# Sachin-A/TraceWeaver

Hardware: NVIDIA H100
Metric: spans/sec reconstructed (in+out spans of all solved services) (higher is better)
Workload: dtype int64 timestamps, f64 log-likelihoods

## Files before the change

### traceweaver_b200/csrc/tw_api.cu

```cuda
#include <cuda_runtime.h>

#include <cstdio>
#include <cstdlib>
#include <cstring>
#include <memory>
#include <random>
#include <string>
#include <vector>

#include "tw_kernels.cuh"

using namespace tw;

static thread_local std::string g_last_error;

static int fail(int code, const char* fmt, const char* a = "", const char* b2 = "") {
  char buf[512];
  snprintf(buf, sizeof buf, fmt, a, b2);
  g_last_error = buf;
  return code;
}

#define CU(expr)                                                                      \
  do {                                                                                \
// ... 52 lines not shown
  DevBuf<int32_t> truth_tab;
  DevBuf<int64_t> truth_tab_off;
  DevBuf<int32_t> in_prob;
  DevBuf<int> order_missing;
  DevBuf<uint8_t> acc_flags;
  DevBuf<unsigned long long> acc_first;
  DevBuf<uint32_t> skip_sets;
  DevBuf<int64_t> skip_set_off;
  DevBuf<uint32_t> skip_taken;
  DevBuf<int32_t> skip_win;
  DevBuf<int32_t> unit_prob;
  DevBuf<int32_t> unit_lo;
  DevBuf<int32_t> unit_hi;
  DevBuf<int> unit_count;
  int max_units = 0;
  DevBuf<int32_t> long_seg;
  int n_long = 0;
  DevBuf<int64_t> long_scratch;
  int64_t slab_len = 1;
  DevBuf<int64_t> in_end_sorted;
  DevBuf<int64_t> out_end_sorted;
  DevBuf<int32_t> batch_prob;
  DevBuf<int32_t> batch_idx;
  int n_batches_total = 0;
  DevBuf<int32_t> term_ep;
  DevBuf<int32_t> ep_prob;
  bool shifted = false;
  DevBuf<int64_t> fixed_times;
  DevBuf<int32_t> prob_shift;
  DevBuf<int32_t> prob_top;
// ... 186 lines not shown
  CU(up(eng->term_ep.p, term_ep));
  CU(up(eng->ep_prob.p, ep_prob));
  CU(cudaStreamSynchronize(s));

  {
    int64_t mu = 0;
    for (int p = 0; p < P; ++p) mu += (h->prob_in_off[p + 1] - h->prob_in_off[p]) / kStitchUnitMin + 1;
    if (mu > 0x7fffffff) return fail(TW_ERR_RANGE_LIMIT, "bind: too many stitch units");
    eng->max_units = (int)mu;
    CU(eng->unit_prob.reserve((size_t)mu));
    CU(eng->unit_lo.reserve((size_t)mu));
    CU(eng->unit_hi.reserve((size_t)mu));
    CU(eng->unit_count.reserve(1));
  }
  {
    std::vector<int32_t> long_seg;
    int64_t longest = 0;
    for (int p = 0; p < P; ++p) {
      const int64_t n = h->prob_in_off[p + 1] - h->prob_in_off[p];
      if (n > kSortSmemCap) { long_seg.push_back(p); longest = n > longest ? n : longest; }
    }
    for (int ep = 0; ep < h->n_ep_total; ++ep) {
      const int64_t n = h->ep_out_off[ep + 1] - h->ep_out_off[ep];
      if (n > kSortSmemCap) { long_seg.push_back(P + ep); longest = n > longest ? n : longest; }
      if (n > eng->max_seg) eng->max_seg = (int)n;
    }
    if (longest > (int64_t)1 << 28) return fail(TW_ERR_RANGE_LIMIT, "bind: a list has more than 2^28 spans");
    eng->n_long = (int)long_seg.size();
    eng->slab_len = 1;
    while (eng->slab_len < longest) eng->slab_len <<= 1;
// ... 333 lines not shown
    return fail(TW_ERR_INVALID, "tw_stitch: params, cut, assign, mis_rank, n_cand are required");
  if (out->topk_score && (!out->topk_idx || !out->topk_cnt)) return fail(TW_ERR_INVALID, "tw_stitch: partial topk outputs");
  tw_score_out spec;
  memset(&spec, 0, sizeof spec);
  if (undeleted) {
    if (!undeleted->topk_score || !undeleted->topk_idx || !undeleted->topk_cnt || !undeleted->n_feasible ||
        !undeleted->used_lo || !undeleted->used_bits || !undeleted->used_wide)
      return fail(TW_ERR_INVALID, "tw_stitch: `undeleted` needs top-K, n_feasible and the used maps");
    spec = *undeleted;
  }
  tw_params sp;
  rc = scoring_params(eng, params, sp, (cudaStream_t)stream);
  if (rc) return rc;
  StitchUnits ub{eng->unit_prob.p, eng->unit_lo.p, eng->unit_hi.p, eng->unit_count.p};
  CU(launch_stitch(eng->dev, sp, cut, spec, *out, eng->taken.p, eng->taken_words, eng->node_limit, ub,
                   eng->max_units, eng->err_flag.p, (cudaStream_t)stream, eng->launches));
  return TW_OK;
}

int tw_delays(tw_engine* eng, const int32_t* assign, const int64_t* term_sample_off, double* delays,
              int32_t* counts, void* stream) {
  int rc = need_bound(eng, "tw_delays");
  if (rc) return rc;
  CU(launch_delays(eng->dev, assign, term_sample_off, eng->term_ep.p, eng->ep_prob.p, delays, counts,
                   eng->shifted ? eng->prob_shift.p : nullptr, (cudaStream_t)stream, eng->launches));
  return TW_OK;
}

static void numpy_random_samples(uint32_t seed, int count, std::vector<double>& out) {
  std::mt19937 mt(seed);
  out.resize(count);
// ... 78 lines not shown
```

### traceweaver_b200/csrc/tw_core.cuh

```cuda
#pragma once
#include <stdint.h>
#include <string.h>
#include <math.h>

#include "../../include/traceweaver_b200.h"

#if defined(__CUDACC__)
#define TW_HD __host__ __device__ __forceinline__
#define TW_HD_NOINLINE __host__ __device__
#else
#define TW_HD inline
#define TW_HD_NOINLINE
#endif

#define TW_MAX_TERMS 48
#define TW_LOG_SQRT_2PI 0.91893853320467274178032973640562
#define TW_LOG_2PI 1.8378770664093453

namespace tw {

#if defined(__CUDA_ARCH__)
TW_HD double dmul(double a, double b) { return __dmul_rn(a, b); }
TW_HD double dadd(double a, double b) { return __dadd_rn(a, b); }
TW_HD double dsub(double a, double b) { return __dsub_rn(a, b); }
// ... 533 lines not shown
    int ai = wi + ws;
    if (ai >= W) break;
    uint32_t a = A[ai] >> bs;
    if (bs && ai + 1 < W) a |= A[ai + 1] << (32 - bs);
    if (a & B[wi]) return true;
  }
  return false;
}

struct WindowBuf {
  double score[TW_WINDOW_CAP][TW_K];
  int idx[TW_WINDOW_CAP][TW_K][TW_MAX_E];
  int cnt[TW_WINDOW_CAP];
  int chosen[TW_WINDOW_CAP];
  uint32_t adj[TW_WINDOW_CAP];
};

TW_HD bool tuples_conflict(const int* a, const int* b, int E) {
  for (int e = 0; e < E; ++e)
    if (a[e] == b[e]) return true;
  return false;
}

TW_HD uint32_t window_adjacency(const WindowBuf& wb, int E, int nw, int k) {
  uint32_t m = 0;
  for (int a = 0; a < nw; ++a) {
    if (a == k) continue;
    bool hit = false;
    for (int r = 0; r < wb.cnt[k] && !hit; ++r)
      for (int q = 0; q < wb.cnt[a] && !hit; ++q)
        hit = tuples_conflict(wb.idx[k][r], wb.idx[a][q], E);
    if (hit) m |= 1u << a;
  }
  return m;
}

#define TW_ASSIGN_MAX_COLS (TW_WINDOW_CAP * (TW_K + 1) + 1)
constexpr int kMwisPricedMin = 7;
constexpr int kMwisSimpleBudget = 1024;
TW_HD_NOINLINE inline void assignment_solve(const WindowBuf& wb, const int* member, int m, int pos, int* best,
                                            double (*price)[TW_K], double* price_total) {
  int colid[TW_WINDOW_CAP * TW_K];
  int ncol = 0;
  short ecol[TW_WINDOW_CAP][TW_K];
  for (int l = 0; l < m; ++l) {
    const int k = member[l];
    for (int r = 0; r < TW_K; ++r) {
      ecol[l][r] = -1;
      if (r >= wb.cnt[k] || !(TW_WEIGHT_OFFSET + wb.score[k][r] > 0.0)) continue;
      const int span = wb.idx[k][r][pos];
      int j = 0;
      while (j < ncol && colid[j] != span) ++j;
      if (j == ncol) colid[ncol++] = span;
      ecol[l][r] = (short)(j + 1);
    }
  }
  const int M = ncol + m;
  double u[TW_WINDOW_CAP + 1], vv[TW_ASSIGN_MAX_COLS], minv[TW_ASSIGN_MAX_COLS];
  short p[TW_ASSIGN_MAX_COLS], way[TW_ASSIGN_MAX_COLS];
  bool used[TW_ASSIGN_MAX_COLS];
  for (int i = 0; i <= m; ++i) u[i] = 0.0;
  for (int j = 0; j <= M; ++j) { vv[j] = 0.0; p[j] = 0; way[j] = 0; }
  const double INF = 1e300;
  for (int i = 1; i <= m; ++i) {
    p[0] = (short)i;
// ... 107 lines not shown
          } else {
            p[freed] = (short)(l + 1);
          }
        }
      }
      if (ok) {
        fixedc[j] = true;
        best[l] = r < TW_K ? r : -1;
        break;
      }
    }
  }
}

#define TW_MWIS_MAX_DEFERRED 4
TW_HD_NOINLINE inline long long mwis_solve(WindowBuf& wb, int E, int nw, long long node_limit,
                                           uint32_t* deferred = nullptr, int* n_deferred = nullptr) {
  long long nodes = 0;
  if (n_deferred) *n_deferred = 0;
  uint32_t todo = nw >= 32 ? 0xffffffffu : ((1u << nw) - 1u);
  for (int k = 0; k < nw; ++k) wb.chosen[k] = -1;
  while (todo) {
    int seed = 0;
    while (!(todo >> seed & 1u)) ++seed;
    uint32_t comp = 1u << seed, frontier = comp;
    while (frontier) {
      int k = 0;
      while (!(frontier >> k & 1u)) ++k;
      frontier &= ~(1u << k);
      uint32_t nb = wb.adj[k] & ~comp;
      comp |= nb;
// ... 56 lines not shown
        }
        int r = iter[level]++;
        if (r > wb.cnt[k]) { --level; continue; }
        if (r == wb.cnt[k]) {
          choice[level] = -1;
          cur[level + 1] = cur[level];
          ++level;
          iter[level] = 0;
          continue;
        }
        double w = TW_WEIGHT_OFFSET + wb.score[k][r];
        if (!(w > 0.0)) continue;
        bool ok = true;
        for (int l = 0; l < level && ok; ++l)
          if (choice[l] >= 0 && (wb.adj[k] >> member[l] & 1u) &&
              tuples_conflict(wb.idx[k][r], wb.idx[member[l]][choice[l]], E))
            ok = false;
        if (!ok) continue;
        choice[level] = r;
        cur[level + 1] = cur[level] + w;
        ++level;
        iter[level] = 0;
      }

      if (simple_done) {
        for (int l = 0; l < m; ++l) wb.chosen[member[l]] = best[l];
        continue;
      }
    }
    if (deferred && *n_deferred < TW_MWIS_MAX_DEFERRED) {
      deferred[(*n_deferred)++] = comp;
// ... 1 lines not shown
    }
#ifdef __CUDA_ARCH__
    return -1;
#else
    uint8_t avail[TW_WINDOW_CAP + 1][TW_WINDOW_CAP];
    double rem[TW_WINDOW_CAP + 1];
    double price[TW_WINDOW_CAP][TW_K];
    double remp[TW_WINDOW_CAP + 1], lam[TW_WINDOW_CAP + 1];
    const bool priced = m >= kMwisPricedMin;
    if (priced) {
      int pos = 0, fewest = 0x7fffffff;
      for (int e = 0; e < E; ++e) {
        int distinct = 0;
        for (int l = 0; l < m; ++l)
          for (int r = 0; r < wb.cnt[member[l]]; ++r) {
            const int sp = wb.idx[member[l]][r][e];
            bool seen = false;
            for (int l2 = 0; l2 <= l && !seen; ++l2)
              for (int r2 = 0; r2 < (l2 < l ? wb.cnt[member[l2]] : r) && !seen; ++r2)
                seen = wb.idx[member[l2]][r2][e] == sp;
            distinct += !seen;
          }
        if (distinct < fewest) { fewest = distinct; pos = e; }
      }
      assignment_solve(wb, member, m, pos, nullptr, price, &lam[0]);
      nodes += m;
    } else {
      lam[0] = 0.0;
      for (int l = 0; l < m; ++l)
        for (int r = 0; r < TW_K; ++r) price[l][r] = 0.0;
    }
    auto best_avail = [&](int j, uint8_t mask) {
      if (!mask) return 0.0;
      int r = 0;
      while (!(mask >> r & 1u)) ++r;
// ... 58 lines not shown
        rem[level + 1] = rem[level] - best_avail(level, avail[level][level]);
        remp[level + 1] = remp[level] - best_reduced(level, avail[level][level]);
        lam[level + 1] = lam[level];
        ++level;
        iter[level] = 0;
        continue;
      }
      if (!(avail[level][level] >> r & 1u)) continue;
      const double w = TW_WEIGHT_OFFSET + wb.score[k][r];
      double rest = 0.0, restp = 0.0;
      for (int j = level + 1; j < m; ++j) {
        uint8_t mask = avail[level][j];
        if (mask && (wb.adj[k] >> member[j] & 1u)) {
          const int kj = member[j];
          for (int q = 0; q < wb.cnt[kj]; ++q)
            if ((mask >> q & 1u) && tuples_conflict(wb.idx[k][r], wb.idx[kj][q], E)) mask &= (uint8_t)~(1u << q);
        }
        avail[level + 1][j] = mask;
        rest += best_avail(j, mask);
        if (priced) restp += best_reduced(j, mask);
      }
      choice[level] = r;
      cur[level + 1] = cur[level] + w;
      rem[level + 1] = rest;
      remp[level + 1] = restp;
      lam[level + 1] = lam[level] - price[level][r];
      ++level;
      iter[level] = 0;
    }
    for (int l = 0; l < m; ++l) wb.chosen[member[l]] = best[l];
#endif
// ... 22 lines not shown
```

### traceweaver_b200/csrc/tw_kernels.cuh

```cuda
#pragma once
#include <cuda_runtime.h>
#include <stdint.h>

#include "tw_core.cuh"

namespace tw {

constexpr int kS3Threads = 128;
constexpr int kS3Tile = 128;
constexpr int kStageSpans = 1536;
constexpr int kTblCap = 3072;
#ifndef TW_WARP_TBL_CAP
#define TW_WARP_TBL_CAP 256
#endif
constexpr int kWarpTblCap = TW_WARP_TBL_CAP;
constexpr int kRedoCoopCombos = 256;
constexpr int kStitchCoopCombos = 512;
constexpr int kTakenWords = 256;
constexpr int kNarrowW = 2;
constexpr int kWideW = 64;
constexpr int kWideThreads = 32;

constexpr int kStitchWarps = 2;

struct TileList {
  const int32_t* tile_prob;
  const int32_t* tile_start;
  int n_tiles;
  int tile_len;
  const int32_t* tile_cnt = nullptr;
};

struct ScoreTiles {
  const int32_t* tile_prob;
  const int32_t* tile_start;
  const int32_t* tile_win;
  uint8_t* overflow;
  int n_tiles;
// ... 18 lines not shown
cudaError_t launch_cut(const tw_batch& b, const tw_score_out& out, const ScoreTiles& st, const int32_t* prev_idx,
                       cudaStream_t s, int64_t& launches);
cudaError_t launch_score_redo(const tw_batch& b, const tw_params* prm, const tw_score_out& out,
                              const TileList& wide, const int32_t* prev_idx, uint8_t* tile_overflow,
                              int n_sm, int* err_flag, cudaStream_t s, int64_t& launches);
struct StitchUnits {
  int32_t* prob;
  int32_t* lo;
  int32_t* hi;
  int* count;
};
constexpr int kStitchUnitMin = 48;
constexpr int kStitchUnitMaxServices = 4096;
cudaError_t launch_stitch(const tw_batch& b, const tw_params& prm, const uint8_t* cut,
                          const tw_score_out& spec, const tw_pass_out& out, uint32_t* taken_words, size_t taken_n_words,
                          long long node_limit, const StitchUnits& unit_buf, int max_units, int* err_flag,
                          cudaStream_t s, int64_t& launches);
constexpr int kSortSmemCap = 16384;
cudaError_t launch_sort_ends(const tw_batch& b, int64_t* in_end_sorted, int64_t* out_end_sorted,
                             int max_seg, const int32_t* long_seg, int n_long, int64_t* long_scratch,
                             int64_t slab_len, int* err_flag, cudaStream_t s, int64_t& launches);
cudaError_t launch_params0(const tw_batch& b, const int64_t* in_end_sorted,
                           const int64_t* out_end_sorted, const int64_t* prob_gauss_off,
                           const int32_t* batch_prob, const int32_t* batch_idx, int n_batches_total,
                           double* gauss_out, const int32_t* prob_shift, cudaStream_t s, int64_t& launches);
cudaError_t launch_delays(const tw_batch& b, const int32_t* assign, const int64_t* term_sample_off,
                          const int32_t* term_ep, const int32_t* ep_prob, double* delays,
                          int32_t* counts, const int32_t* prob_shift, cudaStream_t s, int64_t& launches);

constexpr int kShiftInvalid = 1 << 30;
constexpr int kFixedBits = 55;
struct TimesF64 {
// ... 64 lines not shown
```

### traceweaver_b200/csrc/tw_stitch.cu

```cuda
#include "tw_kernels.cuh"

namespace tw {

#ifdef TW_PROFILE_PHASES
__device__ unsigned long long g_stitch_phase[16];
#define TW_SPHASE(k)                                                                 \
  do {                                                                               \
    if (lane == 0) {                                                                 \
      long long _now = clock64();                                                    \
      atomicAdd(&g_stitch_phase[k], (unsigned long long)(_now - _sp_t0));            \
      _sp_t0 = _now;                                                                 \
    }                                                                                \
  } while (0)
#define TW_SCOUNT(k, v) do { if (lane == 0) atomicAdd(&g_stitch_phase[k], (unsigned long long)(v)); } while (0)
#else
#define TW_SPHASE(k) do { } while (0)
#define TW_SCOUNT(k, v) do { } while (0)
#endif

__device__ __forceinline__ void prefetch_l1(const void* p) {
  asm volatile("prefetch.global.L1 [%0];" ::"l"(p));
}

struct StitchWarpSmem {
  ProbView v;
  WindowBuf wb;
  double tbl[kWarpTblCap];
  uint32_t tk[kTakenWords];
  uint32_t tmp[kTakenWords];
  uint8_t sid[kWarpTblCap];
  uint32_t cconf[32];
  double cw[32];
};

constexpr int kSmallWindow = 6;
constexpr int kSmallSpace = 4096;
__device__ __forceinline__ bool stitch_small_window(StitchWarpSmem& sm, int E, int nw, int lane, long long* nodes_out) {
  WindowBuf& wb = sm.wb;
  const unsigned kAll = 0xffffffffu;
  const int k = lane / TW_K, r = lane - TW_K * k;
  const bool valid = k < nw && r < wb.cnt[k];
  const unsigned vmask = __ballot_sync(kAll, valid);
  uint32_t conf = 0u;
  if (valid) {
    for (int e = 0; e < E; ++e) conf |= __match_any_sync(vmask, wb.idx[k][r][e]);
    conf &= ~(0x1fu << (TW_K * k));
  }
  sm.cconf[lane] = conf;
  sm.cw[lane] = valid ? TW_WEIGHT_OFFSET + wb.score[k][r] : 0.0;
  uint32_t am = 0u;
#pragma unroll
  for (int a = 0; a < kSmallWindow; ++a)
    if ((conf >> (TW_K * a)) & 0x1fu) am |= 1u << a;
  if (lane < nw) { wb.adj[lane] = 0u; wb.chosen[lane] = -1; }
  __syncwarp();
  if (am) atomicOr(&wb.adj[k], am);
  __syncwarp();
  int cnt[kSmallWindow];
  uint32_t adj[kSmallWindow];
#pragma unroll
// ... 71 lines not shown
      for (int a = 0; a < kSmallWindow; ++a) {
        if ((comp >> a) & 1u) {
          const int d = rem / stride[a];
          rem -= d * stride[a];
          if (lane == 0) wb.chosen[a] = d < cnt[a] ? d : -1;
        }
      }
    }
    nodes += space;
  }
  *nodes_out = nodes;
  return true;
}


__device__ __noinline__ long long mwis_component_warp(WindowBuf& wb, int E, uint32_t comp, double* price ,
                                                      long long node_limit, long long nodes, int lane) {
  const unsigned kAll = 0xffffffffu;
  const int m = __popc(comp);
  int kmine = -1;
  {
    uint32_t c = comp;
    for (int l = 0; l < m; ++l) {
      const int k = __ffs(c) - 1;
      c &= c - 1u;
      if (l == lane) kmine = k;
    }
  }
  double lam0 = 0.0;
  if (lane == 0) {
    int member[TW_WINDOW_CAP];
    {
      uint32_t c = comp;
      for (int l = 0; l < m; ++l) { member[l] = __ffs(c) - 1; c &= c - 1u; }
    }
    int pos = 0, fewest = 0x7fffffff;
    for (int e = 0; e < E; ++e) {
      int distinct = 0;
      for (int l = 0; l < m; ++l)
        for (int r = 0; r < wb.cnt[member[l]]; ++r) {
          const int sp = wb.idx[member[l]][r][e];
          bool seen = false;
          for (int l2 = 0; l2 <= l && !seen; ++l2)
            for (int r2 = 0; r2 < (l2 < l ? wb.cnt[member[l2]] : r) && !seen; ++r2)
              seen = wb.idx[member[l2]][r2][e] == sp;
          distinct += !seen;
        }
      if (distinct < fewest) { fewest = distinct; pos = e; }
    }
    assignment_solve(wb, member, m, pos, nullptr, reinterpret_cast<double(*)[TW_K]>(price), &lam0);
  }
  __syncwarp();
  lam0 = __shfl_sync(kAll, lam0, 0);
  nodes += m;
  const bool mine = lane < m;
  const int cnt = mine ? wb.cnt[kmine] : 0;
  double w0 = 0, w1 = 0, w2 = 0, w3 = 0, w4 = 0, q0 = 0, q1 = 0, q2 = 0, q3 = 0, q4 = 0;
  uint8_t av[TW_WINDOW_CAP + 1];
  {
    uint8_t mask = 0;
// ... 62 lines not shown
      if (lane == level) myc = -1;
      av[level + 1] = avmine;
      cur[level + 1] = cur[level];
      rem[level + 1] = rem[level] - ob;
      remp[level + 1] = remp[level] - obp;
      lam[level + 1] = lam[level];
      ++level;
      iter[level] = 0;
      continue;
    }
    if (!(avL >> r & 1u)) continue;
    const int kL = __shfl_sync(kAll, kmine, level);
    uint8_t mask = avmine;
    if (mine && lane > level && mask && (wb.adj[kL] >> kmine & 1u)) {
      for (int q = 0; q < cnt; ++q)
        if ((mask >> q & 1u) && tuples_conflict(wb.idx[kL][r], wb.idx[kmine][q], E)) mask &= (uint8_t)~(1u << q);
    }
    av[level + 1] = mask;
    const bool later = mine && lane > level;
    const double rest = wsum(later ? best_avail(mask) : 0.0);
    const double restp = wsum(later ? best_reduced(mask) : 0.0);
    if (lane == level) myc = r;
    cur[level + 1] = cur[level] + (TW_WEIGHT_OFFSET + wb.score[kL][r]);
    rem[level + 1] = rest;
    remp[level + 1] = restp;
    lam[level + 1] = lam[level] - price[level * TW_K + r];
    ++level;
    iter[level] = 0;
  }
  if (mine) wb.chosen[kmine] = bestc;
  __syncwarp();
  return nodes;
}

__device__ __noinline__ void stitch_search_lanes(StitchWarpSmem& sm, const tw_params& prm, const tw_pass_out& out,
                                                 uint32_t* const* tk_base, const OutWin* w,
                                                 const double* gauss_base, const double* mix_base, const double* etab,
                                                 int E, int lane, int ws, int i, int64_t in_s, int64_t in_e,
                                                 bool todo, int batch0) {
  const ProbView& v = sm.v;
  WindowBuf& wb = sm.wb;
  auto is_taken = [&](int e, int o) {
    return (reinterpret_cast<volatile const uint32_t*>(tk_base[e])[o >> 5] >> (o & 31)) & 1u;
  };
  const bool active = todo, fast = false;
  int lo[TW_MAX_E], r[TW_MAX_E], lo_abs[TW_MAX_E];
  int tsize = 0;
  if (active && !fast) {
    for (int e = 0; e < E; ++e) {
      lo[e] = lower_bound(w[e].s, w[e].n, in_s);
      lo_abs[e] = lo[e];
      r[e] = range_len(w[e], lo[e], in_e);
    }
    tsize = term_table_size(v, r);
  }
  const int brel = i / TW_PARAM_BATCH - batch0;
  auto publish = [&](const TopK& tk, int leaves) {
    const int64_t gi = v.in_off + i;
    out.n_cand[gi] = leaves;
    wb.cnt[lane] = tk.n;
    for (int k = 0; k < tk.n; ++k) {
      wb.score[lane][k] = tk.score[k];
      for (int e = 0; e < E; ++e) wb.idx[lane][k][e] = tk.idx[k][e];
    }
    if (out.topk_score) {
      out.topk_cnt[gi] = (uint8_t)tk.n;
      int32_t* ix = out.topk_idx + TW_K * (v.tuple_off + (int64_t)i * E);
      for (int k = 0; k < TW_K; ++k) {
        out.topk_score[gi * TW_K + k] = k < tk.n ? tk.score[k] : __longlong_as_double(0x7ff8000000000000LL);
        for (int e = 0; e < E; ++e) ix[k * E + e] = k < tk.n ? tk.idx[k][e] : -1;
      }
    }
  };
  bool pending = active;
  {
    const long long Pown = pending ? combo_count(v, r) : 0;
    unsigned heavy = __ballot_sync(0xffffffffu, pending && tsize <= kWarpTblCap && Pown > kStitchCoopCombos &&
                                                    Pown < (1LL << 31));
    while (heavy) {
      const int L = __ffs(heavy) - 1;
      heavy &= heavy - 1u;
      int lo_b[TW_MAX_E], r_b[TW_MAX_E], o_last_b[TW_MAX_E];
      for (int e = 0; e < E; ++e) {
        lo_b[e] = __shfl_sync(0xffffffffu, lo[e], L);
        r_b[e] = __shfl_sync(0xffffffffu, r[e], L);
      }
      const int tsz = __shfl_sync(0xffffffffu, tsize, L);
      const int brel_b = __shfl_sync(0xffffffffu, brel, L);
      const long long P_b = __shfl_sync(0xffffffffu, Pown, L);
      term_table_last_offsets(v, r_b, o_last_b);
      if (lane == L) term_table_fill(v, in_s, in_e, w, lo, r, o_last_b, brel_b, is_taken, sm.tbl, sm.sid);
      __syncwarp();
      for (int sl = lane; sl < tsz; sl += 32) {
        const uint8_t id = sm.sid[sl];
        if (id != TW_SLOT_INVALID) {
          ParamView pv;
          pv.mode = prm.mode;
          pv.gauss = gauss_base ? gauss_base + (int64_t)(batch0 + (id >> 6)) * v.n_terms * TW_GAUSS_REC : nullptr;
          pv.mix = mix_base;
          pv.etab = etab;
          sm.tbl[sl] = term_logpdf(pv, id & 63, sm.tbl[sl]);
        }
      }
      __syncwarp();
      TopK part;
      part.clear();
      int leaves = 0;
      bool tie = false;
      enumerate_combos(v, w, lo_b, r_b, o_last_b, sm.sid, lane, 32, P_b,
                       [&](const int* c, const int64_t* ce, long long) {
                         ++leaves;
                         const double sc = table_score(v, r_b, lo_b, sm.tbl, c, ce);
                         for (int k = 0; k < part.n; ++k) tie = tie || part.score[k] == sc;
                         tie = tie || sc != sc;
                         topk_offer_sorted(v, part, sc, c);
                       });
#pragma unroll
      for (int d = 16; d > 0; d >>= 1) leaves += __shfl_xor_sync(0xffffffffu, leaves, d);
      TopK tkc;
      tkc.clear();
      int head = 0;
      double prev = 0.0;
      for (int round = 0; round <= TW_K; ++round) {
        const double hs = head < part.n ? part.score[head] : -INFINITY;
        double mx = hs;
#pragma unroll
        for (int d = 16; d > 0; d >>= 1) {
// ... 27 lines not shown
    int my = pending ? tsize : 0, incl = my;
#pragma unroll
    for (int d = 1; d < 32; d <<= 1) {
      int o = __shfl_up_sync(0xffffffffu, incl, d);
      if (lane >= d) incl += o;
    }
    const int offset = incl - my;
    const bool lazy = pending && offset == 0 && tsize > kWarpTblCap;
    const bool in_round = pending && !lazy && offset + tsize <= kWarpTblCap;
    int total = in_round ? offset + tsize : 0;
#pragma unroll
    for (int d = 16; d > 0; d >>= 1) total = max(total, __shfl_xor_sync(0xffffffffu, total, d));
    int o_last[TW_MAX_E];
    if (in_round) {
      term_table_last_offsets(v, r, o_last);
      term_table_fill(v, in_s, in_e, w, lo, r, o_last, brel, is_taken, sm.tbl + offset, sm.sid + offset);
    }
    if (lazy) {
      ParamView pv;
      pv.mode = prm.mode;
      pv.gauss = gauss_base ? gauss_base + (int64_t)(i / TW_PARAM_BATCH) * v.n_terms * TW_GAUSS_REC : nullptr;
      pv.mix = mix_base;
      pv.etab = etab;
      TopK tk;
      tk.clear();
      int leaves = 0;
      enumerate(v, in_s, in_e, w, lo, is_taken,
                [&](const int* c, const int64_t* cs, const int64_t* ce) {
                  if (leaves < 0x7fffffff) ++leaves;
                  topk_offer(v, tk, score_tuple(v, pv, in_s, in_e, cs, ce), c);
                });
      topk_finish(v, tk);
      publish(tk, leaves);
      pending = false;
    }
    __syncwarp();
    for (int s = lane; s < total; s += 32) {
      const uint8_t id = sm.sid[s];
      if (id != TW_SLOT_INVALID) {
        ParamView pv;
        pv.mode = prm.mode;
        pv.gauss = gauss_base ? gauss_base + (int64_t)(batch0 + (id >> 6)) * v.n_terms * TW_GAUSS_REC : nullptr;
        pv.mix = mix_base;
        pv.etab = etab;
        sm.tbl[s] = term_logpdf(pv, id & 63, sm.tbl[s]);
      }
    }
    __syncwarp();
    if (in_round) {
      const double* tbl = sm.tbl + offset;
      const uint8_t* sid = sm.sid + offset;
      TopK tk;
      tk.clear();
      int leaves = 0;
      enumerate(v, in_s, in_e, w, lo,
                [&](int e, int o) { return sid[o_last[e] + (o - lo_abs[e])] == TW_SLOT_INVALID; },
                [&](const int* c, const int64_t*, const int64_t* ce) {
                  if (leaves < 0x7fffffff) ++leaves;
                  topk_offer(v, tk, table_score(v, r, lo_abs, tbl, c, ce), c);
                });
      topk_finish(v, tk);
      publish(tk, leaves);
      pending = false;
    }
    if (!__any_sync(0xffffffffu, pending)) break;
    __syncwarp();
  }
  __syncwarp();

}

__device__ __noinline__ long long stitch_mwis_large(StitchWarpSmem& sm, int E, int nw, long long node_limit, int lane) {
  WindowBuf& wb = sm.wb;
  long long nodes = 1;
  __syncwarp();
  if (lane < nw) wb.adj[lane] = window_adjacency(wb, E, nw, lane);
  __syncwarp();
  uint32_t deferred[TW_MWIS_MAX_DEFERRED];
  int n_def = 0;
  if (lane == 0) nodes = mwis_solve(wb, E, nw, node_limit, deferred, &n_def);
  nodes = __shfl_sync(0xffffffffu, nodes, 0);
  n_def = __shfl_sync(0xffffffffu, n_def, 0);
  for (int d = 0; d < n_def && nodes >= 0; ++d) {
    const uint32_t comp = __shfl_sync(0xffffffffu, lane == 0 ? deferred[d] : 0u, 0);
    __syncwarp();
    nodes = mwis_component_warp(wb, E, comp, sm.tbl, node_limit, nodes, lane);
  }
  return nodes;
}

__global__ void __launch_bounds__(kStitchWarps * 32, 10)
k_stitch(tw_batch b, tw_params prm, const uint8_t* __restrict__ cut_all, tw_score_out spec, tw_pass_out out,
         uint32_t* __restrict__ taken, long long node_limit, StitchUnits units, int* __restrict__ err_flag) {
  extern __shared__ __align__(16) unsigned char smem_raw[];
  __shared__ double etab[64];
  load_exp_table(etab);
  const int warp_in_block = threadIdx.x >> 5;
  const int lane = threadIdx.x & 31;
  const int u = blockIdx.x * kStitchWarps + warp_in_block;
  int p, u0 = 0, u1 = -1;
  if (units.prob) {
    if (u >= *units.count) return;
    p = units.prob[u];
    u0 = units.lo[u];
    u1 = units.hi[u];
  } else {
    p = u;
    if (p >= b.n_problems) return;
  }
  StitchWarpSmem& sm = reinterpret_cast<StitchWarpSmem*>(smem_raw)[warp_in_block];
#ifdef TW_PROFILE_PHASES
  long long _sp_t0 = clock64();
#endif
  int rc = TW_OK;
  if (lane == 0) rc = load_view(b, p, sm.v);
  rc = __shfl_sync(0xffffffffu, rc, 0);
  __syncwarp();
  if (rc != TW_OK) {
    if (lane == 0) { atomicMin(err_flag, rc); if (out.counters) out.counters[p * 4 + 3] = rc; }
    return;
  }
  const ProbView& v = sm.v;
  WindowBuf& wb = sm.wb;
  const int n = v.n_in, E = v.E;
  if (u1 < 0) u1 = n;
  const uint8_t* cut = cut_all + v.in_off;

  uint32_t* tk_base[TW_MAX_E];
  OutWin w[TW_MAX_E];
  int tk_words = 0;
  for (int e = 0; e < E; ++e) tk_words += (v.n_out[e] >> 5) + 3;
  const bool tk_smem = tk_words <= kTakenWords;
  {
    int off = 0;
    for (int e = 0; e < E; ++e) {
      tk_base[e] = tk_smem ? sm.tk + off : taken + (v.out_off[e] >> 5) + (v.ep0 + e);
      off += (v.n_out[e] >> 5) + 3;
      w[e].s = v.os[e]; w[e].e = v.oe[e]; w[e].base = 0; w[e].n = v.n_out[e];
    }
  }
  if (tk_smem)
    for (int x = lane; x < tk_words; x += 32) { sm.tk[x] = 0u; sm.tmp[x] = 0u; }
  __syncwarp();
  for (int i = u0 + lane; i < u1; i += 32) {
    out.mis_rank[v.in_off + i] = -1;
    for (int e = 0; e < E; ++e) out.assign[v.tuple_off + (int64_t)e * n + i] = -1;
  }

  const double* gauss_base = prm.mode == TW_PARAMS_GAUSS_BATCHED
                                 ? prm.gauss + prm.prob_gauss_off[p] * TW_GAUSS_REC : nullptr;
  const double* mix_base = prm.mode == TW_PARAMS_MIXTURE ? prm.mix + (int64_t)v.term0 * TW_MIX_REC : nullptr;

  WindowCursor wc;
  wc.init();
  int not_best = 0, unassigned = 0;
  long long max_nodes = 0;
  int ws = u0;
// ... 31 lines not shown
        const bool act = lane < R;
        const int ir = ws + (act ? lane : 0);
        const int64_t gi = v.in_off + ir;
        const int64_t base = v.tuple_off + (int64_t)ir * E;
        bool ok = act ? spec.used_wide[gi] == 0 : true;
        if (act && ok) {
          for (int e = 0; e < E; ++e) {
            const int ulo = spec.used_lo[base + e];
            const uint32_t u0 = spec.used_bits[2 * (base + e)], u1 = spec.used_bits[2 * (base + e) + 1];
            if ((u0 | u1) == 0u) continue;
            const int q = ulo >> 5, sh = ulo & 31;
            const uint32_t m0 = u0 << sh;
            const uint32_t m1 = sh ? (u0 >> (32 - sh)) | (u1 << sh) : u1;
            const uint32_t m2 = sh ? (u1 >> (32 - sh)) : 0u;
            uint32_t* tkp = tk_base[e] + q;
            uint32_t* tmp = sm.tmp + (tkp - sm.tk);
            if ((tkp[0] & m0) | (tkp[1] & m1) | (tkp[2] & m2)) ok = false;
            if (m0 && (atomicOr(&tmp[0], m0) & m0)) ok = false;
            if (m1 && (atomicOr(&tmp[1], m1) & m1)) ok = false;
            if (m2 && (atomicOr(&tmp[2], m2) & m2)) ok = false;
          }
        }
        const bool all_ok = __all_sync(0xffffffffu, ok);
        __syncwarp();
        if (act && spec.used_wide[gi] == 0) {
          for (int e = 0; e < E; ++e) {
            const int ulo = spec.used_lo[base + e];
            uint32_t* tmp = sm.tmp + ((tk_base[e] + (ulo >> 5)) - sm.tk);
            tmp[0] = 0u; tmp[1] = 0u; tmp[2] = 0u;
          }
        }
        __syncwarp();
        TW_SPHASE(2);
        if (all_ok) {
          int rank = -2;
          if (act) {
            const int cnt = spec.topk_cnt[gi];
            rank = (cnt > 0 && TW_WEIGHT_OFFSET + spec.topk_score[gi * TW_K] > 0.0) ? 0 : -1;
            out.n_cand[gi] = spec.n_feasible[gi];
            out.mis_rank[gi] = (int8_t)rank;
            if (rank == 0) {
              const int32_t* ix = spec.topk_idx + TW_K * base;
              for (int e = 0; e < E; ++e) {
// ... 64 lines not shown
        const uint32_t a = tkw[0], bq = tkw[1], c2 = tkw[2];
        hit |= __funnelshift_r(a, bq, sh) & u0;
        hit |= __funnelshift_r(bq, c2, sh) & u1;
      }
      fast = hit == 0u;
    }
    const int batch0 = ws / TW_PARAM_BATCH;
    if (fast) {
      const int64_t gi = v.in_off + i;
      const int cnt = spec.topk_cnt[gi];
      out.n_cand[gi] = spec.n_feasible[gi];
      wb.cnt[lane] = cnt;
      const int32_t* ix = spec.topk_idx + TW_K * (v.tuple_off + (int64_t)i * E);
      for (int k = 0; k < cnt; ++k) {
        wb.score[lane][k] = spec.topk_score[gi * TW_K + k];
        for (int e = 0; e < E; ++e) wb.idx[lane][k][e] = ix[k * E + e];
      }
      if (out.topk_score) {
        out.topk_cnt[gi] = (uint8_t)cnt;
        int32_t* ox = out.topk_idx + TW_K * (v.tuple_off + (int64_t)i * E);
        for (int k = 0; k < TW_K; ++k) {
          out.topk_score[gi * TW_K + k] = spec.topk_score[gi * TW_K + k];
          for (int e = 0; e < E; ++e) ox[k * E + e] = ix[k * E + e];
        }
      }
    }
    TW_SPHASE(5);
    const unsigned slow_mask = __ballot_sync(0xffffffffu, active && !fast);
    TW_SCOUNT(14, __popc(slow_mask));
    if (slow_mask)
      stitch_search_lanes(sm, prm, out, tk_base, w, gauss_base, mix_base, etab, E, lane, ws, i, in_s, in_e,
                          active && !fast, batch0);
    __syncwarp();
    TW_SPHASE(6);
    long long nodes = 1;
    if (nw == 1) {
      if (lane == 0) wb.chosen[0] = (wb.cnt[0] > 0 && TW_WEIGHT_OFFSET + wb.score[0][0] > 0.0) ? 0 : -1;
    } else {
      bool solved = false;
      if (nw <= kSmallWindow) solved = stitch_small_window(sm, E, nw, lane, &nodes);
      if (!solved) {
        nodes = stitch_mwis_large(sm, E, nw, node_limit, lane);
      }
    }
    __syncwarp();
    TW_SPHASE(7);
    if (nodes < 0) { rc = TW_ERR_MWIS_LIMIT; break; }
    if (nodes > max_nodes) max_nodes = nodes;
    int rank = -2;
    if (lane < nw) {
      rank = wb.chosen[lane];
      out.mis_rank[v.in_off + i] = (int8_t)rank;
      if (rank >= 0) {
        for (int e = 0; e < E; ++e) {
          int o = wb.idx[lane][rank][e];
          out.assign[v.tuple_off + (int64_t)e * n + i] = o;
          atomicOr(&tk_base[e][o >> 5], 1u << (o & 31));
        }
      }
    }
    not_best += __popc(__ballot_sync(0xffffffffu, lane < nw && rank != 0));
    unassigned += __popc(__ballot_sync(0xffffffffu, lane < nw && rank < 0));
    if (!tk_smem) __threadfence_block();
    __syncwarp();
    ws = we + 1;
    TW_SPHASE(8);
  }
  if (lane == 0) {
    if (rc != TW_OK) atomicMin(err_flag, rc);
    if (out.counters) {
// ... 73 lines not shown
  emit(unit_start, n);
}

#ifdef TW_PROFILE_PHASES
extern "C" int tw_debug_stitch_phases(unsigned long long* out16, int reset) {
  cudaError_t e = cudaMemcpyFromSymbol(out16, g_stitch_phase, sizeof(unsigned long long) * 16);
  if (e != cudaSuccess) return -2;
  if (reset) {
    unsigned long long z[16] = {0};
    cudaMemcpyToSymbol(g_stitch_phase, z, sizeof z);
  }
  return 0;
}
#endif

cudaError_t setup_stitch() {
  return cudaFuncSetAttribute(k_stitch, cudaFuncAttributeMaxDynamicSharedMemorySize,
                              (int)(sizeof(StitchWarpSmem) * kStitchWarps));
}

cudaError_t launch_stitch(const tw_batch& b, const tw_params& prm, const uint8_t* cut,
                          const tw_score_out& spec, const tw_pass_out& out, uint32_t* taken_words, size_t taken_n_words,
                          long long node_limit, const StitchUnits& unit_buf, int max_units, int* err_flag,
                          cudaStream_t s, int64_t& launches) {
  cudaError_t e = cudaMemsetAsync(taken_words, 0, taken_n_words * sizeof(uint32_t), s);
  if (e != cudaSuccess) return e;
  if (out.counters) {
    e = cudaMemsetAsync(out.counters, 0, (size_t)b.n_problems * 4 * sizeof(int32_t), s);
    if (e != cudaSuccess) return e;
  }
  size_t smem = sizeof(StitchWarpSmem) * kStitchWarps;
  StitchUnits units{nullptr, nullptr, nullptr, nullptr};
  int warps = b.n_problems;
  if (spec.used_lo && unit_buf.prob && max_units > 0 && b.n_problems < kStitchUnitMaxServices) {
    units = unit_buf;
    e = cudaMemsetAsync(units.count, 0, sizeof(int), s);
    if (e != cudaSuccess) return e;
    k_stitch_units<<<(b.n_problems + 3) / 4, 128, 0, s>>>(b, cut, spec, kStitchUnitMin, units);
    e = after_launch(launches);
    if (e != cudaSuccess) return e;
    warps = max_units;
  }
  int blocks = (warps + kStitchWarps - 1) / kStitchWarps;
  k_stitch<<<blocks, kStitchWarps * 32, smem, s>>>(b, prm, cut, spec, out, taken_words, node_limit, units, err_flag);
  return after_launch(launches);
}

}
```

Baseline: 438.7 million.

## Shrink stitch shared memory with runtime-sized slabs and global scratch tables

The per-warp shared-memory block of the stitch kernel is reorganized. The term tables move to a global-memory scratch array, the taken/tmp bitmaps are sized from the bound workload, and the window buffer is repacked by endpoint so only the needed endpoint columns are allocated. Launch bounds now target more blocks per SM. The goal is higher occupancy on the latency-bound stitch kernel, at the cost of term-table accesses going to global memory and a possible register squeeze from the higher launch-bounds target.

Result: faster. 456.1 million, median of 6 (+4.0%).

```diff
diff --git a/traceweaver_b200/csrc/tw_api.cu b/traceweaver_b200/csrc/tw_api.cu
--- a/traceweaver_b200/csrc/tw_api.cu
+++ b/traceweaver_b200/csrc/tw_api.cu
@@ -90,6 +90,8 @@
   DevBuf<int32_t> unit_hi;
   DevBuf<int> unit_count;
   int max_units = 0;
+  StitchLayout stitch_layout{};
+  DevBuf<StitchTables> stitch_tables;
   DevBuf<int32_t> long_seg;
   int n_long = 0;
   DevBuf<int64_t> long_scratch;
@@ -306,6 +308,18 @@
     CU(eng->unit_count.reserve(1));
   }
   {
+    int e_max = 1, tk_max = 0;
+    for (int p = 0; p < P; ++p) {
+      const int ep0 = h->prob_ep_off[p], E = h->prob_ep_off[p + 1] - ep0;
+      int tk = 0;
+      for (int e = 0; e < E; ++e) tk += (int)((h->ep_out_off[ep0 + e + 1] - h->ep_out_off[ep0 + e]) >> 5) + 3;
+      e_max = E > e_max ? E : e_max;
+      tk_max = tk > tk_max ? tk : tk_max;
+    }
+    eng->stitch_layout = stitch_layout(e_max, tk_max);
+    CU(eng->stitch_tables.reserve((size_t)(P > eng->max_units ? P : eng->max_units) + kStitchWarps));
+  }
+  {
     std::vector<int32_t> long_seg;
     int64_t longest = 0;
     for (int p = 0; p < P; ++p) {
@@ -669,7 +683,8 @@
   if (rc) return rc;
   StitchUnits ub{eng->unit_prob.p, eng->unit_lo.p, eng->unit_hi.p, eng->unit_count.p};
   CU(launch_stitch(eng->dev, sp, cut, spec, *out, eng->taken.p, eng->taken_words, eng->node_limit, ub,
-                   eng->max_units, eng->err_flag.p, (cudaStream_t)stream, eng->launches));
+                   eng->max_units, eng->stitch_layout, eng->stitch_tables.p, eng->err_flag.p, (cudaStream_t)stream,
+                   eng->launches));
   return TW_OK;
 }
 
diff --git a/traceweaver_b200/csrc/tw_core.cuh b/traceweaver_b200/csrc/tw_core.cuh
--- a/traceweaver_b200/csrc/tw_core.cuh
+++ b/traceweaver_b200/csrc/tw_core.cuh
@@ -571,6 +571,21 @@
   int cnt[TW_WINDOW_CAP];
   int chosen[TW_WINDOW_CAP];
   uint32_t adj[TW_WINDOW_CAP];
+  TW_HD int& at(int k, int r, int e) { return idx[k][r][e]; }
+  TW_HD int at(int k, int r, int e) const { return idx[k][r][e]; }
+};
+
+struct PackedWindowBuf {
+  double score[TW_WINDOW_CAP][TW_K];
+  int cnt[TW_WINDOW_CAP];
+  int chosen[TW_WINDOW_CAP];
+  uint32_t adj[TW_WINDOW_CAP];
+  int idx[TW_MAX_E][TW_WINDOW_CAP * TW_K];
+  TW_HD int& at(int k, int r, int e) { return idx[e][k * TW_K + r]; }
+  TW_HD int at(int k, int r, int e) const { return idx[e][k * TW_K + r]; }
+  static constexpr int packed_bytes(int e_max) {
+    return (int)(sizeof(PackedWindowBuf) - sizeof(int) * TW_WINDOW_CAP * TW_K * (TW_MAX_E - e_max));
+  }
 };
 
 TW_HD bool tuples_conflict(const int* a, const int* b, int E) {
@@ -579,14 +594,22 @@
   return false;
 }
 
-TW_HD uint32_t window_adjacency(const WindowBuf& wb, int E, int nw, int k) {
+template <class WB>
+TW_HD bool cands_conflict(const WB& wb, int k, int r, int a, int q, int E) {
+  for (int e = 0; e < E; ++e)
+    if (wb.at(k, r, e) == wb.at(a, q, e)) return true;
+  return false;
+}
+
+template <class WB>
+TW_HD uint32_t window_adjacency(const WB& wb, int E, int nw, int k) {
   uint32_t m = 0;
   for (int a = 0; a < nw; ++a) {
     if (a == k) continue;
     bool hit = false;
     for (int r = 0; r < wb.cnt[k] && !hit; ++r)
       for (int q = 0; q < wb.cnt[a] && !hit; ++q)
-        hit = tuples_conflict(wb.idx[k][r], wb.idx[a][q], E);
+        hit = cands_conflict(wb, k, r, a, q, E);
     if (hit) m |= 1u << a;
   }
   return m;
@@ -595,7 +618,8 @@
 #define TW_ASSIGN_MAX_COLS (TW_WINDOW_CAP * (TW_K + 1) + 1)
 constexpr int kMwisPricedMin = 7;
 constexpr int kMwisSimpleBudget = 1024;
-TW_HD_NOINLINE inline void assignment_solve(const WindowBuf& wb, const int* member, int m, int pos, int* best,
+template <class WB>
+TW_HD_NOINLINE inline void assignment_solve(const WB& wb, const int* member, int m, int pos, int* best,
                                             double (*price)[TW_K], double* price_total) {
   int colid[TW_WINDOW_CAP * TW_K];
   int ncol = 0;
@@ -605,7 +629,7 @@
     for (int r = 0; r < TW_K; ++r) {
       ecol[l][r] = -1;
       if (r >= wb.cnt[k] || !(TW_WEIGHT_OFFSET + wb.score[k][r] > 0.0)) continue;
-      const int span = wb.idx[k][r][pos];
+      const int span = wb.at(k, r, pos);
       int j = 0;
       while (j < ncol && colid[j] != span) ++j;
       if (j == ncol) colid[ncol++] = span;
@@ -743,7 +767,8 @@
 }
 
 #define TW_MWIS_MAX_DEFERRED 4
-TW_HD_NOINLINE inline long long mwis_solve(WindowBuf& wb, int E, int nw, long long node_limit,
+template <class WB>
+TW_HD_NOINLINE inline long long mwis_solve(WB& wb, int E, int nw, long long node_limit,
                                            uint32_t* deferred = nullptr, int* n_deferred = nullptr) {
   long long nodes = 0;
   if (n_deferred) *n_deferred = 0;
@@ -830,7 +855,7 @@
         bool ok = true;
         for (int l = 0; l < level && ok; ++l)
           if (choice[l] >= 0 && (wb.adj[k] >> member[l] & 1u) &&
-              tuples_conflict(wb.idx[k][r], wb.idx[member[l]][choice[l]], E))
+              cands_conflict(wb, k, r, member[l], choice[l], E))
             ok = false;
         if (!ok) continue;
         choice[level] = r;
@@ -862,11 +887,11 @@
         int distinct = 0;
         for (int l = 0; l < m; ++l)
           for (int r = 0; r < wb.cnt[member[l]]; ++r) {
-            const int sp = wb.idx[member[l]][r][e];
+            const int sp = wb.at(member[l], r, e);
             bool seen = false;
             for (int l2 = 0; l2 <= l && !seen; ++l2)
               for (int r2 = 0; r2 < (l2 < l ? wb.cnt[member[l2]] : r) && !seen; ++r2)
-                seen = wb.idx[member[l2]][r2][e] == sp;
+                seen = wb.at(member[l2], r2, e) == sp;
             distinct += !seen;
           }
         if (distinct < fewest) { fewest = distinct; pos = e; }
@@ -955,7 +980,7 @@
         if (mask && (wb.adj[k] >> member[j] & 1u)) {
           const int kj = member[j];
           for (int q = 0; q < wb.cnt[kj]; ++q)
-            if ((mask >> q & 1u) && tuples_conflict(wb.idx[k][r], wb.idx[kj][q], E)) mask &= (uint8_t)~(1u << q);
+            if ((mask >> q & 1u) && cands_conflict(wb, k, r, kj, q, E)) mask &= (uint8_t)~(1u << q);
         }
         avail[level + 1][j] = mask;
         rest += best_avail(j, mask);
diff --git a/traceweaver_b200/csrc/tw_kernels.cuh b/traceweaver_b200/csrc/tw_kernels.cuh
--- a/traceweaver_b200/csrc/tw_kernels.cuh
+++ b/traceweaver_b200/csrc/tw_kernels.cuh
@@ -22,6 +22,19 @@
 constexpr int kWideThreads = 32;
 
 constexpr int kStitchWarps = 2;
+constexpr int kStitchBlocksPerSM = 14;
+
+struct StitchTables {
+  double tbl[kWarpTblCap];
+  uint8_t sid[kWarpTblCap];
+};
+
+struct StitchLayout {
+  int tk_words;
+  int wb_off;
+  int bytes;
+};
+StitchLayout stitch_layout(int e_max, int tk_words_max);
 
 struct TileList {
   const int32_t* tile_prob;
@@ -70,8 +83,8 @@
 constexpr int kStitchUnitMaxServices = 4096;
 cudaError_t launch_stitch(const tw_batch& b, const tw_params& prm, const uint8_t* cut,
                           const tw_score_out& spec, const tw_pass_out& out, uint32_t* taken_words, size_t taken_n_words,
-                          long long node_limit, const StitchUnits& unit_buf, int max_units, int* err_flag,
-                          cudaStream_t s, int64_t& launches);
+                          long long node_limit, const StitchUnits& unit_buf, int max_units, const StitchLayout& layout,
+                          StitchTables* tables, int* err_flag, cudaStream_t s, int64_t& launches);
 constexpr int kSortSmemCap = 16384;
 cudaError_t launch_sort_ends(const tw_batch& b, int64_t* in_end_sorted, int64_t* out_end_sorted,
                              int max_seg, const int32_t* long_seg, int n_long, int64_t* long_scratch,
diff --git a/traceweaver_b200/csrc/tw_stitch.cu b/traceweaver_b200/csrc/tw_stitch.cu
--- a/traceweaver_b200/csrc/tw_stitch.cu
+++ b/traceweaver_b200/csrc/tw_stitch.cu
@@ -24,26 +24,31 @@
 
 struct StitchWarpSmem {
   ProbView v;
-  WindowBuf wb;
-  double tbl[kWarpTblCap];
-  uint32_t tk[kTakenWords];
-  uint32_t tmp[kTakenWords];
-  uint8_t sid[kWarpTblCap];
   uint32_t cconf[32];
   double cw[32];
 };
+static_assert(sizeof(StitchWarpSmem) % 8 == 0, "the taken bitmaps and the window buffer follow 8-byte aligned");
+
+struct StitchSlab {
+  unsigned char* base;
+  __device__ StitchWarpSmem& fixed() const { return *reinterpret_cast<StitchWarpSmem*>(base); }
+  __device__ uint32_t* taken() const { return reinterpret_cast<uint32_t*>(base + sizeof(StitchWarpSmem)); }
+  __device__ PackedWindowBuf& window(const StitchLayout& L) const {
+    return *reinterpret_cast<PackedWindowBuf*>(base + L.wb_off);
+  }
+};
 
 constexpr int kSmallWindow = 6;
 constexpr int kSmallSpace = 4096;
-__device__ __forceinline__ bool stitch_small_window(StitchWarpSmem& sm, int E, int nw, int lane, long long* nodes_out) {
-  WindowBuf& wb = sm.wb;
+__device__ __forceinline__ bool stitch_small_window(StitchWarpSmem& sm, PackedWindowBuf& wb, int E, int nw, int lane,
+                                                    long long* nodes_out) {
   const unsigned kAll = 0xffffffffu;
   const int k = lane / TW_K, r = lane - TW_K * k;
   const bool valid = k < nw && r < wb.cnt[k];
   const unsigned vmask = __ballot_sync(kAll, valid);
   uint32_t conf = 0u;
   if (valid) {
-    for (int e = 0; e < E; ++e) conf |= __match_any_sync(vmask, wb.idx[k][r][e]);
+    for (int e = 0; e < E; ++e) conf |= __match_any_sync(vmask, wb.at(k, r, e));
     conf &= ~(0x1fu << (TW_K * k));
   }
   sm.cconf[lane] = conf;
@@ -145,7 +150,7 @@
 }
 
 
-__device__ __noinline__ long long mwis_component_warp(WindowBuf& wb, int E, uint32_t comp, double* price ,
+__device__ __noinline__ long long mwis_component_warp(PackedWindowBuf& wb, int E, uint32_t comp, double* price ,
                                                       long long node_limit, long long nodes, int lane) {
   const unsigned kAll = 0xffffffffu;
   const int m = __popc(comp);
@@ -170,11 +175,11 @@
       int distinct = 0;
       for (int l = 0; l < m; ++l)
         for (int r = 0; r < wb.cnt[member[l]]; ++r) {
-          const int sp = wb.idx[member[l]][r][e];
+          const int sp = wb.at(member[l], r, e);
           bool seen = false;
           for (int l2 = 0; l2 <= l && !seen; ++l2)
             for (int r2 = 0; r2 < (l2 < l ? wb.cnt[member[l2]] : r) && !seen; ++r2)
-              seen = wb.idx[member[l2]][r2][e] == sp;
+              seen = wb.at(member[l2], r2, e) == sp;
           distinct += !seen;
         }
       if (distinct < fewest) { fewest = distinct; pos = e; }
@@ -267,7 +272,7 @@
     uint8_t mask = avmine;
     if (mine && lane > level && mask && (wb.adj[kL] >> kmine & 1u)) {
       for (int q = 0; q < cnt; ++q)
-        if ((mask >> q & 1u) && tuples_conflict(wb.idx[kL][r], wb.idx[kmine][q], E)) mask &= (uint8_t)~(1u << q);
+        if ((mask >> q & 1u) && cands_conflict(wb, kL, r, kmine, q, E)) mask &= (uint8_t)~(1u << q);
     }
     av[level + 1] = mask;
     const bool later = mine && lane > level;
@@ -286,13 +291,12 @@
   return nodes;
 }
 
-__device__ __noinline__ void stitch_search_lanes(StitchWarpSmem& sm, const tw_params& prm, const tw_pass_out& out,
+__device__ __noinline__ void stitch_search_lanes(const ProbView& v, PackedWindowBuf& wb, StitchTables& tb,
+                                                 const tw_params& prm, const tw_pass_out& out,
                                                  uint32_t* const* tk_base, const OutWin* w,
                                                  const double* gauss_base, const double* mix_base, const double* etab,
                                                  int E, int lane, int ws, int i, int64_t in_s, int64_t in_e,
                                                  bool todo, int batch0) {
-  const ProbView& v = sm.v;
-  WindowBuf& wb = sm.wb;
   auto is_taken = [&](int e, int o) {
     return (reinterpret_cast<volatile const uint32_t*>(tk_base[e])[o >> 5] >> (o & 31)) & 1u;
   };
@@ -314,7 +318,7 @@
     wb.cnt[lane] = tk.n;
     for (int k = 0; k < tk.n; ++k) {
       wb.score[lane][k] = tk.score[k];
-      for (int e = 0; e < E; ++e) wb.idx[lane][k][e] = tk.idx[k][e];
+      for (int e = 0; e < E; ++e) wb.at(lane, k, e) = tk.idx[k][e];
     }
     if (out.topk_score) {
       out.topk_cnt[gi] = (uint8_t)tk.n;
@@ -342,17 +346,17 @@
       const int brel_b = __shfl_sync(0xffffffffu, brel, L);
       const long long P_b = __shfl_sync(0xffffffffu, Pown, L);
       term_table_last_offsets(v, r_b, o_last_b);
-      if (lane == L) term_table_fill(v, in_s, in_e, w, lo, r, o_last_b, brel_b, is_taken, sm.tbl, sm.sid);
+      if (lane == L) term_table_fill(v, in_s, in_e, w, lo, r, o_last_b, brel_b, is_taken, tb.tbl, tb.sid);
       __syncwarp();
       for (int sl = lane; sl < tsz; sl += 32) {
-        const uint8_t id = sm.sid[sl];
+        const uint8_t id = tb.sid[sl];
         if (id != TW_SLOT_INVALID) {
           ParamView pv;
           pv.mode = prm.mode;
           pv.gauss = gauss_base ? gauss_base + (int64_t)(batch0 + (id >> 6)) * v.n_terms * TW_GAUSS_REC : nullptr;
           pv.mix = mix_base;
           pv.etab = etab;
-          sm.tbl[sl] = term_logpdf(pv, id & 63, sm.tbl[sl]);
+          tb.tbl[sl] = term_logpdf(pv, id & 63, tb.tbl[sl]);
         }
       }
       __syncwarp();
@@ -360,10 +364,10 @@
       part.clear();
       int leaves = 0;
       bool tie = false;
-      enumerate_combos(v, w, lo_b, r_b, o_last_b, sm.sid, lane, 32, P_b,
+      enumerate_combos(v, w, lo_b, r_b, o_last_b, tb.sid, lane, 32, P_b,
                        [&](const int* c, const int64_t* ce, long long) {
                          ++leaves;
-                         const double sc = table_score(v, r_b, lo_b, sm.tbl, c, ce);
+                         const double sc = table_score(v, r_b, lo_b, tb.tbl, c, ce);
                          for (int k = 0; k < part.n; ++k) tie = tie || part.score[k] == sc;
                          tie = tie || sc != sc;
                          topk_offer_sorted(v, part, sc, c);
@@ -421,7 +425,7 @@
     int o_last[TW_MAX_E];
     if (in_round) {
       term_table_last_offsets(v, r, o_last);
-      term_table_fill(v, in_s, in_e, w, lo, r, o_last, brel, is_taken, sm.tbl + offset, sm.sid + offset);
+      term_table_fill(v, in_s, in_e, w, lo, r, o_last, brel, is_taken, tb.tbl + offset, tb.sid + offset);
     }
     if (lazy) {
       ParamView pv;
@@ -443,20 +447,20 @@
     }
     __syncwarp();
     for (int s = lane; s < total; s += 32) {
-      const uint8_t id = sm.sid[s];
+      const uint8_t id = tb.sid[s];
       if (id != TW_SLOT_INVALID) {
         ParamView pv;
         pv.mode = prm.mode;
         pv.gauss = gauss_base ? gauss_base + (int64_t)(batch0 + (id >> 6)) * v.n_terms * TW_GAUSS_REC : nullptr;
         pv.mix = mix_base;
         pv.etab = etab;
-        sm.tbl[s] = term_logpdf(pv, id & 63, sm.tbl[s]);
+        tb.tbl[s] = term_logpdf(pv, id & 63, tb.tbl[s]);
       }
     }
     __syncwarp();
     if (in_round) {
-      const double* tbl = sm.tbl + offset;
-      const uint8_t* sid = sm.sid + offset;
+      const double* tbl = tb.tbl + offset;
+      const uint8_t* sid = tb.sid + offset;
       TopK tk;
       tk.clear();
       int leaves = 0;
@@ -477,8 +481,8 @@
 
 }
 
-__device__ __noinline__ long long stitch_mwis_large(StitchWarpSmem& sm, int E, int nw, long long node_limit, int lane) {
-  WindowBuf& wb = sm.wb;
+__device__ __noinline__ long long stitch_mwis_large(PackedWindowBuf& wb, StitchTables& tb, int E, int nw,
+                                                   long long node_limit, int lane) {
   long long nodes = 1;
   __syncwarp();
   if (lane < nw) wb.adj[lane] = window_adjacency(wb, E, nw, lane);
@@ -491,14 +495,15 @@
   for (int d = 0; d < n_def && nodes >= 0; ++d) {
     const uint32_t comp = __shfl_sync(0xffffffffu, lane == 0 ? deferred[d] : 0u, 0);
     __syncwarp();
-    nodes = mwis_component_warp(wb, E, comp, sm.tbl, node_limit, nodes, lane);
+    nodes = mwis_component_warp(wb, E, comp, tb.tbl, node_limit, nodes, lane);
   }
   return nodes;
 }
 
-__global__ void __launch_bounds__(kStitchWarps * 32, 10)
+__global__ void __launch_bounds__(kStitchWarps * 32, kStitchBlocksPerSM)
 k_stitch(tw_batch b, tw_params prm, const uint8_t* __restrict__ cut_all, tw_score_out spec, tw_pass_out out,
-         uint32_t* __restrict__ taken, long long node_limit, StitchUnits units, int* __restrict__ err_flag) {
+         uint32_t* __restrict__ taken, long long node_limit, StitchUnits units, StitchLayout layout,
+         StitchTables* __restrict__ tables, int* __restrict__ err_flag) {
   extern __shared__ __align__(16) unsigned char smem_raw[];
   __shared__ double etab[64];
   load_exp_table(etab);
@@ -515,7 +520,8 @@
     p = u;
     if (p >= b.n_problems) return;
   }
-  StitchWarpSmem& sm = reinterpret_cast<StitchWarpSmem*>(smem_raw)[warp_in_block];
+  const StitchSlab slab{smem_raw + warp_in_block * layout.bytes};
+  StitchWarpSmem& sm = slab.fixed();
 #ifdef TW_PROFILE_PHASES
   long long _sp_t0 = clock64();
 #endif
@@ -528,7 +534,7 @@
     return;
   }
   const ProbView& v = sm.v;
-  WindowBuf& wb = sm.wb;
+  PackedWindowBuf& wb = slab.window(layout);
   const int n = v.n_in, E = v.E;
   if (u1 < 0) u1 = n;
   const uint8_t* cut = cut_all + v.in_off;
@@ -537,17 +543,18 @@
   OutWin w[TW_MAX_E];
   int tk_words = 0;
   for (int e = 0; e < E; ++e) tk_words += (v.n_out[e] >> 5) + 3;
-  const bool tk_smem = tk_words <= kTakenWords;
+  const bool tk_smem = tk_words <= layout.tk_words;
+  uint32_t* const tk_slab = slab.taken();
   {
     int off = 0;
     for (int e = 0; e < E; ++e) {
-      tk_base[e] = tk_smem ? sm.tk + off : taken + (v.out_off[e] >> 5) + (v.ep0 + e);
+      tk_base[e] = tk_smem ? tk_slab + off : taken + (v.out_off[e] >> 5) + (v.ep0 + e);
       off += (v.n_out[e] >> 5) + 3;
       w[e].s = v.os[e]; w[e].e = v.oe[e]; w[e].base = 0; w[e].n = v.n_out[e];
     }
   }
   if (tk_smem)
-    for (int x = lane; x < tk_words; x += 32) { sm.tk[x] = 0u; sm.tmp[x] = 0u; }
+    for (int x = lane; x < tk_words; x += 32) { tk_slab[x] = 0u; tk_slab[layout.tk_words + x] = 0u; }
   __syncwarp();
   for (int i = u0 + lane; i < u1; i += 32) {
     out.mis_rank[v.in_off + i] = -1;
@@ -609,7 +616,7 @@
             const uint32_t m1 = sh ? (u0 >> (32 - sh)) | (u1 << sh) : u1;
             const uint32_t m2 = sh ? (u1 >> (32 - sh)) : 0u;
             uint32_t* tkp = tk_base[e] + q;
-            uint32_t* tmp = sm.tmp + (tkp - sm.tk);
+            uint32_t* tmp = tkp + layout.tk_words;
             if ((tkp[0] & m0) | (tkp[1] & m1) | (tkp[2] & m2)) ok = false;
             if (m0 && (atomicOr(&tmp[0], m0) & m0)) ok = false;
             if (m1 && (atomicOr(&tmp[1], m1) & m1)) ok = false;
@@ -621,7 +628,7 @@
         if (act && spec.used_wide[gi] == 0) {
           for (int e = 0; e < E; ++e) {
             const int ulo = spec.used_lo[base + e];
-            uint32_t* tmp = sm.tmp + ((tk_base[e] + (ulo >> 5)) - sm.tk);
+            uint32_t* tmp = tk_base[e] + (ulo >> 5) + layout.tk_words;
             tmp[0] = 0u; tmp[1] = 0u; tmp[2] = 0u;
           }
         }
@@ -716,7 +723,7 @@
       const int32_t* ix = spec.topk_idx + TW_K * (v.tuple_off + (int64_t)i * E);
       for (int k = 0; k < cnt; ++k) {
         wb.score[lane][k] = spec.topk_score[gi * TW_K + k];
-        for (int e = 0; e < E; ++e) wb.idx[lane][k][e] = ix[k * E + e];
+        for (int e = 0; e < E; ++e) wb.at(lane, k, e) = ix[k * E + e];
       }
       if (out.topk_score) {
         out.topk_cnt[gi] = (uint8_t)cnt;
@@ -731,7 +738,7 @@
     const unsigned slow_mask = __ballot_sync(0xffffffffu, active && !fast);
     TW_SCOUNT(14, __popc(slow_mask));
     if (slow_mask)
-      stitch_search_lanes(sm, prm, out, tk_base, w, gauss_base, mix_base, etab, E, lane, ws, i, in_s, in_e,
+      stitch_search_lanes(v, wb, tables[u], prm, out, tk_base, w, gauss_base, mix_base, etab, E, lane, ws, i, in_s, in_e,
                           active && !fast, batch0);
     __syncwarp();
     TW_SPHASE(6);
@@ -740,9 +747,10 @@
       if (lane == 0) wb.chosen[0] = (wb.cnt[0] > 0 && TW_WEIGHT_OFFSET + wb.score[0][0] > 0.0) ? 0 : -1;
     } else {
       bool solved = false;
-      if (nw <= kSmallWindow) solved = stitch_small_window(sm, E, nw, lane, &nodes);
+      if (nw <= kSmallWindow) solved = stitch_small_window(sm, wb, E, nw, lane, &nodes);
       if (!solved) {
-        nodes = stitch_mwis_large(sm, E, nw, node_limit, lane);
+        TW_SCOUNT(15, 1);
+        nodes = stitch_mwis_large(wb, tables[u], E, nw, node_limit, lane);
       }
     }
     __syncwarp();
@@ -755,7 +763,7 @@
       out.mis_rank[v.in_off + i] = (int8_t)rank;
       if (rank >= 0) {
         for (int e = 0; e < E; ++e) {
-          int o = wb.idx[lane][rank][e];
+          int o = wb.at(lane, rank, e);
           out.assign[v.tuple_off + (int64_t)e * n + i] = o;
           atomicOr(&tk_base[e][o >> 5], 1u << (o & 31));
         }
@@ -859,22 +867,30 @@
 }
 #endif
 
+StitchLayout stitch_layout(int e_max, int tk_words_max) {
+  StitchLayout L;
+  L.tk_words = tk_words_max < kTakenWords ? tk_words_max : kTakenWords;
+  L.wb_off = (int)sizeof(StitchWarpSmem) + 2 * L.tk_words * (int)sizeof(uint32_t);
+  L.bytes = (L.wb_off + PackedWindowBuf::packed_bytes(e_max) + 15) & ~15;
+  return L;
+}
+
 cudaError_t setup_stitch() {
   return cudaFuncSetAttribute(k_stitch, cudaFuncAttributeMaxDynamicSharedMemorySize,
-                              (int)(sizeof(StitchWarpSmem) * kStitchWarps));
+                              stitch_layout(TW_MAX_E, kTakenWords).bytes * kStitchWarps);
 }
 
 cudaError_t launch_stitch(const tw_batch& b, const tw_params& prm, const uint8_t* cut,
                           const tw_score_out& spec, const tw_pass_out& out, uint32_t* taken_words, size_t taken_n_words,
-                          long long node_limit, const StitchUnits& unit_buf, int max_units, int* err_flag,
-                          cudaStream_t s, int64_t& launches) {
+                          long long node_limit, const StitchUnits& unit_buf, int max_units, const StitchLayout& layout,
+                          StitchTables* tables, int* err_flag, cudaStream_t s, int64_t& launches) {
   cudaError_t e = cudaMemsetAsync(taken_words, 0, taken_n_words * sizeof(uint32_t), s);
   if (e != cudaSuccess) return e;
   if (out.counters) {
     e = cudaMemsetAsync(out.counters, 0, (size_t)b.n_problems * 4 * sizeof(int32_t), s);
     if (e != cudaSuccess) return e;
   }
-  size_t smem = sizeof(StitchWarpSmem) * kStitchWarps;
+  const size_t smem = (size_t)layout.bytes * kStitchWarps;
   StitchUnits units{nullptr, nullptr, nullptr, nullptr};
   int warps = b.n_problems;
   if (spec.used_lo && unit_buf.prob && max_units > 0 && b.n_problems < kStitchUnitMaxServices) {
@@ -887,7 +903,8 @@
     warps = max_units;
   }
   int blocks = (warps + kStitchWarps - 1) / kStitchWarps;
-  k_stitch<<<blocks, kStitchWarps * 32, smem, s>>>(b, prm, cut, spec, out, taken_words, node_limit, units, err_flag);
+  k_stitch<<<blocks, kStitchWarps * 32, smem, s>>>(b, prm, cut, spec, out, taken_words, node_limit, units, layout,
+                                                   tables, err_flag);
   return after_launch(launches);
 }
 
```
